# Pose-Group/FAMI-Pose

Hardware: AMD Instinct MI355X
Metric: train clips/sec (5-frame 384x288 HRNet-W48) (higher is better)
Workload: dtype f32

## Files before the change

fami-pose_amd/csrc/conv.hip:

```cpp
#include "common.h"
#include <type_traits>
#include <string.h>

#include "conv_epi.h"
#include "conv_pair.h"
extern "C" int fami_conv2d_fwd_bnin_ok(int N, int H, int W, int Ci, int Co);
extern "C" int fami_dcn_tune(int mode);
extern "C" int fami_bn_tune_small(long elems);
extern "C" void fami_conv_stem_tune(int on);
int fami_pair_launch(const PairCapture& c, hipStream_t s);
int fami_try_conv_stem1(int half_kind, const void* x, const void* wp, const float* bias, void* y, int N, int H, int W, int Ci, int Co,
                        int kh, int kw, int stride, int pad, int dil, int NTt, int relu, int accumulate, int out_f32, hipStream_t s,
                        const char* name, const EpiBN& epi);


struct ConvArgs {
  EpiBN e;
  int emode;
  const float* x;
  const float* wp;
  float* y;
  const float* bias;
  const float* addend;
  int N, Hi, Wi, Ci, Ho, Wo, Co;
// ... 589 lines not shown
  int xcd;
  int par;
};

template <typename H>
__global__ void pack_w_h_kernel(const float* __restrict__ w, H* __restrict__ wp, int Co, int Ci, int taps,
                                int KC, int NTt, int mode) {
  const long total = (long)taps * KC * NTt * 512;
  for (long i = blockIdx.x * (long)blockDim.x + threadIdx.x; i < total; i += (long)gridDim.x * blockDim.x) {
    const int j = (int)(i & 7), lane = (int)((i >> 3) & 63);
    long r = i >> 9;
    const int nt = (int)(r % NTt);
    r /= NTt;
    const int kc = (int)(r % KC), tap = (int)(r / KC);
    const int kidx = kc * 32 + (lane >> 4) * 8 + j, nidx = nt * 16 + (lane & 15);
    const int co = mode == 0 ? nidx : kidx, ci = mode == 0 ? kidx : nidx;
    float v = 0.f;
    if (co < Co && ci < Ci) v = w[((long)co * Ci + ci) * taps + tap];
    wp[i] = (H)v;
  }
}

struct PackDesc { long src, dst; int Co, Ci, taps, mode; };
template <typename T>
__global__ __launch_bounds__(256) void pack_w_batch_kernel(const float* __restrict__ params, T* __restrict__ packed,
                                                           const PackDesc* __restrict__ desc) {
  const PackDesc d = desc[blockIdx.y];
  const float* w = params + d.src;
  T* wp = packed + d.dst;
  const int kd = d.mode == 0 ? d.Ci : d.Co, nd = d.mode == 0 ? d.Co : d.Ci;
  constexpr int KG = sizeof(T) == 4 ? 16 : 32, FR = sizeof(T) == 4 ? 4 : 8;
  if (d.taps > 1 && d.taps <= 9) {
    __shared__ float tile[32 * (16 * 9 + 1) + 16];
    const int taps = d.taps;
    const int KC = (kd + KG - 1) / KG, NTt = (nd + 15) / 16;
    const int rows = d.mode == 0 ? 16 : KG, cols = d.mode == 0 ? KG : 16;
    const int run = cols * taps, pitch = run + 1;
    for (int b = blockIdx.x; b < KC * NTt; b += gridDim.x) {
      const int kc = b / NTt, nt = b - kc * NTt;
      const int co0 = d.mode == 0 ? nt * 16 : kc * KG, ci0 = d.mode == 0 ? kc * KG : nt * 16;
      __syncthreads();
      for (int i = threadIdx.x; i < rows * run; i += 256) {
        const int r = i / run, c = i - r * run;
        const int co = co0 + r, ci = ci0 + c / taps;
        tile[r * pitch + c] = (co < d.Co && ci < d.Ci) ? w[((long)co * d.Ci + ci0) * taps + c] : 0.f;
      }
      __syncthreads();
      for (int o = threadIdx.x; o < taps * 64 * FR; o += 256) {
        const int tap = o / (64 * FR), within = o - tap * (64 * FR);
        const int lane = within / FR, j = within - lane * FR;
        const int kl = (lane >> 4) * FR + j, nl = lane & 15;
        const int col = d.mode == 0 ? nl : kl, cil = d.mode == 0 ? kl : nl;
        st1(wp + ((long)(tap * KC + kc) * NTt + nt) * (64 * FR) + within, tile[col * pitch + cil * taps + tap]);
      }
    }
    return;
  }
  if constexpr (sizeof(T) == 4) {
    const long total = pack16_elems(kd, nd, d.taps) + pack32_elems(kd, nd, d.taps);
    for (long i = blockIdx.x * (long)blockDim.x + threadIdx.x; i < total; i += (long)gridDim.x * blockDim.x)
      st1(wp + i, pack_f32_elem(w, i, d.Co, d.Ci, d.taps, d.mode));
  } else {
    const int KC = (kd + KG - 1) / KG, NTt = (nd + 15) / 16;
    const long total = (long)d.taps * KC * NTt * 64 * FR;
    for (long i = blockIdx.x * (long)blockDim.x + threadIdx.x; i < total; i += (long)gridDim.x * blockDim.x) {
      const int j = (int)(i % FR), lane = (int)((i / FR) & 63);
      long r = i / (FR * 64);
      const int nt = (int)(r % NTt);
      r /= NTt;
      const int kc = (int)(r % KC), tap = (int)(r / KC);
      const int kidx = kc * KG + (lane >> 4) * FR + j, nidx = nt * 16 + (lane & 15);
      const int co = d.mode == 0 ? nidx : kidx, ci = d.mode == 0 ? kidx : nidx;
      float v = 0.f;
      if (co < d.Co && ci < d.Ci) v = w[((long)co * d.Ci + ci) * d.taps + tap];
      st1(wp + i, v);
    }
// ... 2314 lines not shown
  FAMI_REQUIRE(desc_out, nm, "null descriptor");
  EpiBN e = epi_none();
  if (slots) {
    FAMI_REQUIRE(epi_bwd_stats_ok(z, yrelu, mean, invstd, gamma, beta, relu), nm, "bad argument");
    e = epi_bwd_stats(slots, Ci, z, yrelu, mean, invstd, gamma, beta, relu);
  }
  return bwd_pair_run(
      nm, desc_out, s,
      [&] { return conv_dgrad_h_impl<HT>(nm, dy, wpd, dx, N, H, W, Ci, Co, kh, kw, stride, pad, dil, acc_dx, s, e); },
      [&] { return wgrad_h_impl<HT>(nm, x, dy, dw, workspace, ws_bytes, N, H, W, Ci, Co, kh, kw, stride, pad, dil, acc_dw, s); });
}

extern "C" {

int fami_conv_tune(int mt, int nt, int ks) {
  g_force_mt = mt; g_force_nt = nt; g_force_ks = ks;
  return FAMI_OK;
}
int fami_conv_tune_lds(int on) {
  if (on == 9000 || on == 9001) {
    fami_conv_stem_tune(on - 9000);
    return FAMI_OK;
  }
  if (on < 0) fami_conv_stem_tune(-1);
  if (on == 10 || on == 11 || on == 20 || on == 21 || on == 30 || on == 31 || (on >= 40 && on <= 42) || (on >= 52 && on <= 54) || (on >= 60 && on <= 62) || on >= 100) {
    fami_conv_t4_tune(on);
    return FAMI_OK;
  }
  g_use_lds = on < 0 ? -1 : (on ? 1 : 0);
  g_lds_sim = on == 2;
  if (on < 0) fami_conv_t4_tune(-1);
  return FAMI_OK;
}
int fami_conv_tune_wgrad_lds(int on) {
  if (on >= 30000) {
    fami_wgrad_s3_tune(on - 30000);
    return FAMI_OK;
  }
  if (on >= 20000) {
    fami_wgrad16_tune(on - 20000);
    return FAMI_OK;
  }
  if (on >= 1000) {
    g_wgrad_ps = on - 1000;
    return FAMI_OK;
  }
  if (on >= 50 && on <= 54) {
// ... 59 lines not shown
}

long fami_packed_weight_elems(int Co, int Ci, int kh, int kw, int mode) {
  const int kd = mode == 0 ? Ci : Co, nd = mode == 0 ? Co : Ci;
  return pack16_elems(kd, nd, kh * kw) + pack32_elems(kd, nd, kh * kw) + fami_split_image_elems(kd, nd, kh * kw);
}

int fami_pack_conv_weight_f32(const float* w_oihw, float* wp, int Co, int Ci, int kh, int kw, int mode,
                              hipStream_t s) {
  FAMI_REQUIRE(w_oihw && wp && Co > 0 && Ci > 0 && (mode == 0 || mode == 1), "fami_pack_conv_weight_f32", "bad argument");
  const int kd = mode == 0 ? Ci : Co, nd = mode == 0 ? Co : Ci;
  const long total = pack16_elems(kd, nd, kh * kw) + pack32_elems(kd, nd, kh * kw);
  hipLaunchKernelGGL(pack_w_kernel, dim3(fami_ew_grid(total)), dim3(256), 0, s, w_oihw, wp, Co, Ci, kh * kw, mode);
  FAMI_CHECK_LAUNCH("fami_pack_conv_weight_f32");
  if (fami_split_image_elems(kd, nd, kh * kw) > 0) {
    fami_pack_split_single(w_oihw, wp + total, Co, Ci, kh * kw, mode, s);
    FAMI_CHECK_LAUNCH("fami_pack_conv_weight_f32/split");
  }
  return FAMI_OK;
}

int fami_pack_conv_weights_batch_f32(const float* params, float* packed, const void* desc, int n, hipStream_t s) {
  FAMI_REQUIRE(params && packed && desc && n > 0 && n < 65536, "fami_pack_conv_weights_batch_f32", "bad argument");
  hipLaunchKernelGGL(pack_w_batch_kernel<float>, dim3(48, n), dim3(256), 0, s, params, packed, reinterpret_cast<const PackDesc*>(desc));
  FAMI_CHECK_LAUNCH("fami_pack_conv_weights_batch_f32");
  fami_pack_split_batch(params, packed, desc, n, s);
  FAMI_CHECK_LAUNCH("fami_pack_conv_weights_batch_f32/split");
  return FAMI_OK;
}

int fami_conv2d_fwd_f32(const float* x, const float* wp, const float* bias, const float* addend, float* y, int N,
                        int H, int W, int Ci, int Co, int kh, int kw, int stride, int pad, int dil, int relu,
                        int accumulate, hipStream_t s) {
  return conv_fwd_f32_impl("fami_conv2d_fwd_f32", x, wp, bias, addend, y, N, H, W, Ci, Co, kh, kw, stride, pad, dil, relu,
                           accumulate, epi_none(), s);
}
int fami_conv2d_fwd_stats_f32(const float* x, const float* wp, const float* bias, float* y, int N, int H, int W, int Ci,
                              int Co, int kh, int kw, int stride, int pad, int dil, void* slots, const float* pivot_src,
                              hipStream_t s) {
  FAMI_REQUIRE(slots, "fami_conv2d_fwd_stats_f32", "null slots");
  return conv_fwd_f32_impl("fami_conv2d_fwd_stats_f32", x, wp, bias, nullptr, y, N, H, W, Ci, Co, kh, kw, stride, pad, dil,
                           0, 0, epi_fwd_stats(slots, Co, pivot_src), s);
}
int fami_conv2d_fwd_xbn_f32(const float* z, const float* wp, const float* bias, float* y, int N, int H, int W, int Ci, int Co,
                            void* slots, const float* pivot_src, const void* xslots, long xP, const float* xgamma,
                            const float* xbeta, float* xmean, float* xinvstd, float* xrunning_mean, float* xrunning_var,
// ... 203 lines not shown
```

fami-pose_amd/csrc/conv_epi.h:

```cpp
#pragma once
#include "common.h"

struct EpiBN {
  double* slots;
  int ns, mode, relu, C;
  const float* pivot_src;
  const void* z;
  const void* yr;
  const float *mean, *invstd, *gamma, *beta;
};
static inline EpiBN epi_none() {
  EpiBN e;
  e.slots = nullptr; e.ns = 1; e.mode = 0; e.relu = 0; e.C = 0; e.pivot_src = nullptr; e.z = nullptr; e.yr = nullptr;
  e.mean = e.invstd = e.gamma = e.beta = nullptr;
  return e;
}
static inline EpiBN epi_fwd_stats(void* slots, int Co, const float* pivot_src) {
  EpiBN e = epi_none();
  if (!slots) return e;
  e.slots = reinterpret_cast<double*>(slots); e.ns = bn_slots(Co); e.mode = 1; e.C = Co; e.pivot_src = pivot_src;
  return e;
}
static inline bool epi_bwd_stats_ok(const void* z, const void* yrelu, const float* mean, const float* invstd, const float* gamma,
                                    const float* beta, int relu) {
// ... 97 lines not shown
int fami_try_conv3x3_t4(int half_kind, const void* x, const void* wp, const float* bias, void* y, int N, int H, int W, int Ci,
                        int Co, int KC, int NTt, int sgn, int relu, int accumulate, int out_f32, hipStream_t s,
                        const char* name, const EpiBN& epi, const XBN& xbn = xbn_none());
int fami_try_conv3x3_t4_dil(int half_kind, const void* x, const void* wp, const float* bias, void* y, int N, int H, int W, int Ci,
                            int Co, int KC, int NTt, int sgn, int relu, int accumulate, int out_f32, int dil, hipStream_t s,
                            const char* name);
void fami_conv_t4_tune(int on);
void fami_conv_t4_default_split(int on);
int fami_conv_t4_eligible16(int N, int H, int W, int Ci, int Co);
int fami_conv_t4_eligible_s3(int N, int H, int W, int Ci, int Co);

long fami_wgrad16_slabs(int N, int H, int W, int Ci, int Co, int k, int st, int pad, int dil);
int fami_try_wgrad16(int half_kind, const void* x, const void* dy, float* part, long ws_bytes, int N, int H, int W, int Ci,
                     int Co, int k, int st, int pad, int dil, hipStream_t s, const char* name, const XBN& xbn = xbn_none());
void fami_wgrad16_tune(int on);

long fami_wgrad_s3_slabs(int N, int H, int W, int Ci, int Co);
int fami_try_wgrad_s3(const float* x, const float* dy, float* part, long ws_bytes, int N, int H, int W, int Ci, int Co,
                      hipStream_t s, const char* name, const XBN& xbn = xbn_none());
void fami_wgrad_s3_tune(int on);
void fami_wgrad_s3_default(int on);

long fami_split_image_elems(int kd, int nd, int taps);
void fami_pack_split_single(const float* w_oihw, float* split, int Co, int Ci, int taps, int mode, hipStream_t s);
void fami_pack_split_batch(const float* params, float* packed, const void* desc, int n, hipStream_t s);
int fami_try_conv3x3_t5(int half_kind, const void* x, const void* wp, const float* bias, void* y, int N, int H, int W, int Ci,
                        int Co, int KC, int NTt, int sgn, int relu, int accumulate, int out_f32, hipStream_t s,
                        const char* name, const EpiBN& epi, const XBN& xbn);
void fami_conv_t5_tune(int on);
int fami_conv_t5_eligible_s3(int N, int H, int W, int Ci, int Co);

int fami_try_conv3x3_t6(int half_kind, const void* x, const void* wp, const float* bias, void* y, int N, int H, int W, int Ci,
                        int Co, int KC, int NTt, int sgn, int relu, int accumulate, int out_f32, hipStream_t s,
                        const char* name, const EpiBN& epi, const XBN& xbn);
extern "C" int fami_conv_t6_eligible(int N, int H, int W, int Ci, int Co);
void fami_conv_t6_tune(int on);
```

fami-pose_amd/csrc/conv_t5.hip:

```cpp
#include "conv_epi.h"
#include "conv_t5_dev.h"
#include "conv_pair.h"
#include <type_traits>


long fami_split_image_elems(int kd, int nd, int taps) {
  return (taps == 9 && kd % 16 == 0) ? (long)taps * (kd / 16) * ((nd + 15) / 16) * 384 : 0;
}
__device__ __forceinline__ void t5_split3(float v, __bf16& h0, __bf16& h1, __bf16& h2) {
  h0 = (__bf16)v;
  const float r1 = v - (float)h0;
  h1 = (__bf16)r1;
  const float r2 = r1 - (float)h1;
  h2 = (__bf16)r2;
}
struct T5PackDesc { long src, dst; int Co, Ci, taps, mode; };
__device__ __forceinline__ void t5_pack_split_image(const float* __restrict__ w, __bf16* __restrict__ sp, int Co, int Ci,
                                                    int mode, int first_block, int block_stride, float* tile) {
  const int kd = mode == 0 ? Ci : Co, nd = mode == 0 ? Co : Ci;
  const int KC = kd / 16, NTt = (nd + 15) / 16;
  constexpr int PITCH = 16 * 9 + 1;
  for (int b = first_block; b < KC * NTt; b += block_stride) {
    const int kc = b / NTt, nt = b - kc * NTt;
    const int co0 = mode == 0 ? nt * 16 : kc * 16, ci0 = mode == 0 ? kc * 16 : nt * 16;
    __syncthreads();
    for (int i = threadIdx.x; i < 16 * 144; i += 256) {
      const int r = i / 144, c = i - r * 144;
      const int co = co0 + r, ci = ci0 + c / 9;
      tile[r * PITCH + c] = (co < Co && ci < Ci) ? w[((long)co * Ci + ci0) * 9 + c] : 0.f;
    }
    __syncthreads();
    for (int o = threadIdx.x; o < 9 * 64; o += 256) {
      const int tap = o >> 6, n = (o >> 2) & 15, k4 = (o & 3) * 4;
      t5_bf16x4 h0, h1, h2;
#pragma unroll
      for (int j = 0; j < 4; ++j) {
        const int k = k4 + j;
        const float v = mode == 0 ? tile[n * PITCH + k * 9 + tap] : tile[k * PITCH + n * 9 + tap];
        __bf16 a0, a1, a2;
        t5_split3(v, a0, a1, a2);
        h0[j] = a0; h1[j] = a1; h2[j] = a2;
      }
      __bf16* blk = sp + ((long)(tap * KC + kc) * NTt + nt) * 768 + n * 16 + k4;
      *reinterpret_cast<t5_bf16x4*>(blk) = h0;
      *reinterpret_cast<t5_bf16x4*>(blk + 256) = h1;
      *reinterpret_cast<t5_bf16x4*>(blk + 512) = h2;
    }
  }
}
__global__ __launch_bounds__(256) void t5_pack_split_kernel(const float* __restrict__ w, __bf16* __restrict__ sp, int Co, int Ci, int mode) {
  __shared__ float tile[16 * (16 * 9 + 1)];
  t5_pack_split_image(w, sp, Co, Ci, mode, blockIdx.x, gridDim.x, tile);
}
__global__ __launch_bounds__(256) void t5_pack_split_batch_kernel(const float* __restrict__ params, float* __restrict__ packed,
                                                                   const T5PackDesc* __restrict__ desc) {
  __shared__ float tile[16 * (16 * 9 + 1)];
  const T5PackDesc d = desc[blockIdx.y];
  const int kd = d.mode == 0 ? d.Ci : d.Co, nd = d.mode == 0 ? d.Co : d.Ci;
  if (d.taps != 9 || (kd % 16) != 0) return;
  const long n16 = (long)9 * (kd / 16) * ((nd + 15) / 16) * 256;
  t5_pack_split_image(params + d.src, reinterpret_cast<__bf16*>(packed + d.dst + n16), d.Co, d.Ci, d.mode, blockIdx.x, gridDim.x, tile);
}
void fami_pack_split_single(const float* w_oihw, float* split, int Co, int Ci, int taps, int mode, hipStream_t s) {
  const int kd = mode == 0 ? Ci : Co, nd = mode == 0 ? Co : Ci;
  if (fami_split_image_elems(kd, nd, taps) == 0) return;
  int blocks = (kd / 16) * ((nd + 15) / 16);
  if (blocks > 512) blocks = 512;
  hipLaunchKernelGGL(t5_pack_split_kernel, dim3(blocks), dim3(256), 0, s, w_oihw, reinterpret_cast<__bf16*>(split), Co, Ci, mode);
}
void fami_pack_split_batch(const float* params, float* packed, const void* desc, int n, hipStream_t s) {
// ... 148 lines not shown
```

fami-pose_amd/csrc/conv_t5_dev.h:

```cpp
#pragma once
#include "conv_epi.h"
#include <type_traits>
typedef __bf16 t5_bf16x4 __attribute__((ext_vector_type(4)));

struct ConvT5Args {
  EpiBN e;
  int emode;
  XBN xb;
  const void* x;
  const void* wimg;
  void* y;
  const float* bias;
  int N, H, W, Ci, Co;
  int R, bands, cblocks, njobs;
  int PW, KC, NTt;
  int sgn, relu, accumulate, out_f32;
  int ppl;
  int patch_bytes;
  int nposmax;
  int abl_chunks;
  long long* dbg;
};

#define T5_THREADS 512
#define T5_WAVES 8
#define T5_MTT 3
// ... 481 lines not shown
```

fami-pose_amd/csrc/norm.hip:

```cpp
#include "common.h"

#define BN_MAXG 512
#ifndef BN_U
#define BN_U 4
#endif

struct ColMap {
  int cv, prow, rows, CV;
  bool active;
};
__device__ __forceinline__ ColMap col_map(int C) {
  ColMap m;
  m.CV = C >> 2;
  m.rows = 256 / m.CV;
  m.cv = threadIdx.x % m.CV;
  m.prow = threadIdx.x / m.CV;
  m.active = m.prow < m.rows;
  return m;
}

__device__ __forceinline__ double block_sum_d(double v, double* sm4) {
  v = wave_sum_d(v);
  const int lane = threadIdx.x & 63, wave = threadIdx.x >> 6;
  __syncthreads();
// ... 188 lines not shown
__device__ __forceinline__ f32x4 bn_relu_mask(f32x4 g, f32x4 yy) {
#pragma unroll
  for (int t = 0; t < 4; ++t) g[t] = yy[t] > 0.f ? g[t] : 0.f;
  return g;
}
__device__ __forceinline__ f32x4 bn_relu_mask(f32x4 g, int relu, f32x4 yy, f32x4 xv, f32x4 sc, f32x4 sf) {
  if (relu == 1) return bn_relu_mask(g, yy);
  if (relu == 2) {
#pragma unroll
    for (int t = 0; t < 4; ++t) g[t] = __builtin_fmaf(xv[t], sc[t], sf[t]) > 0.f ? g[t] : 0.f;
  }
  return g;
}

__device__ __forceinline__ void bn_load_stats(const float* __restrict__ mean, const float* __restrict__ invstd, int c0, f32x4& mu,
                                              f32x4& is) {
#pragma unroll
  for (int t = 0; t < 4; ++t) {
    mu[t] = mean[c0 + t];
    is[t] = invstd[c0 + t];
  }
}

template <typename T>
__device__ __forceinline__ void bn_bwd_sums(const T* __restrict__ dy, const T* __restrict__ x, const T* __restrict__ y,
                                            const ColMap& m, long P, int C, int relu, f32x4 mu, f32x4 is, f32x4 sc, f32x4 sf,
                                            f32x4& s, f32x4& q) {
  const long step = (long)gridDim.x * m.rows;
  for (long p = (long)blockIdx.x * m.rows + m.prow; p < P; p += BN_U * step) {
    f32x4 g[BN_U], yy[BN_U], xx[BN_U];
    long o[BN_U];
#pragma unroll
    for (int u = 0; u < BN_U; ++u) {
      const long pu = p + u * step;
      o[u] = (pu < P ? pu : p) * C + m.cv * 4;
      g[u] = ld4(dy + o[u]);
    }
    if (relu & 1) {
#pragma unroll
      for (int u = 0; u < BN_U; ++u) yy[u] = ld4(y + o[u]);
    }
#pragma unroll
    for (int u = 0; u < BN_U; ++u) xx[u] = ld4(x + o[u]);
#pragma unroll
    for (int u = 0; u < BN_U; ++u) {
      if (relu == 1) g[u] = bn_relu_mask(g[u], yy[u]);
      if (relu == 2) g[u] = bn_relu_mask(g[u], relu, yy[u], xx[u], sc, sf);
      if (p + u * step >= P) g[u] = f32x4{0.f, 0.f, 0.f, 0.f};
      const f32x4 xh = (xx[u] - mu) * is;
      s += g[u];
      q += g[u] * xh;
    }
  }
}

template <typename T>
__global__ __launch_bounds__(256) void bn_bwd_partial_kernel(const T* __restrict__ dy,
                                                             const T* __restrict__ x,
                                                             const T* __restrict__ y,
                                                             const float* __restrict__ mean,
                                                             const float* __restrict__ invstd,
                                                             float* __restrict__ partial, long P, int C, int relu) {
  extern __shared__ float sm[];
  const ColMap m = col_map(C);
  f32x4 s = {0.f, 0.f, 0.f, 0.f}, q = {0.f, 0.f, 0.f, 0.f};
  if (m.active) {
    f32x4 mu, is;
    bn_load_stats(mean, invstd, m.cv * 4, mu, is);
    const f32x4 none = {0.f, 0.f, 0.f, 0.f};
    bn_bwd_sums(dy, x, y, m, P, C, relu ? 1 : 0, mu, is, none, none, s, q);
    bn_stage_rows(sm, m, C, s, q);
  }
  bn_fold_rows<false>(sm, m.rows, C, partial, nullptr, 0);
}

__global__ void bn_bwd_finalize_kernel(const float* __restrict__ partial, int G, long P, int C, float* coef,
                                       float* dgamma, float* dbeta, int accumulate) {
  __shared__ double sm4[4];
  const int c = blockIdx.x;
  double s = 0.0, q = 0.0;
  for (int g = threadIdx.x; g < G; g += 256) {
    s += (double)partial[(long)g * 2 * C + c];
    q += (double)partial[(long)g * 2 * C + C + c];
  }
  s = block_sum_d(s, sm4);
  q = block_sum_d(q, sm4);
  if (threadIdx.x != 0) return;
  if (coef) {
    coef[c] = (float)(s / (double)P);
    coef[C + c] = (float)(q / (double)P);
  }
  if (dgamma) dgamma[c] = accumulate ? dgamma[c] + (float)q : (float)q;
  if (dbeta) dbeta[c] = accumulate ? dbeta[c] + (float)s : (float)s;
// ... 148 lines not shown
    bn_scale_shift(muf, isf, gamma[c], beta[c], sc, sf);
    sm[c] = sc;
    sm[C + c] = sf;
  }
  __syncthreads();
  const ColMap m = col_map(C);
  if (!m.active) return;
  const f32x4 sc = *reinterpret_cast<const f32x4*>(sm + m.cv * 4), sf = *reinterpret_cast<const f32x4*>(sm + C + m.cv * 4);
  for (long p = (long)blockIdx.x * m.rows + m.prow; p < P; p += (long)gridDim.x * m.rows) {
    const long o = p * C + m.cv * 4;
    const f32x4 xv = ld4(x + o);
    f32x4 v;
#pragma unroll
    for (int t = 0; t < 4; ++t) v[t] = __builtin_fmaf(xv[t], sc[t], sf[t]);
    if (residual) v += ld4(residual + o);
    if (relu) {
#pragma unroll
      for (int t = 0; t < 4; ++t) v[t] = fmaxf(v[t], 0.f);
    }
    st4(y + o, v);
  }
}

template <typename T>
__global__ __launch_bounds__(256) void bn_bwd_partial2_kernel(const T* __restrict__ dy, const T* __restrict__ x,
                                                              const T* __restrict__ y, const float* __restrict__ mean,
                                                              const float* __restrict__ invstd,
                                                              const float* __restrict__ gamma,
                                                              const float* __restrict__ beta,
                                                              double* __restrict__ slots, int NS, long P, int C, int relu) {
  extern __shared__ float sm[];
  const ColMap m = col_map(C);
  f32x4 s = {0.f, 0.f, 0.f, 0.f}, q = {0.f, 0.f, 0.f, 0.f};
  if (m.active) {
    f32x4 mu, is, sc, sf;
    bn_load_stats(mean, invstd, m.cv * 4, mu, is);
#pragma unroll
    for (int t = 0; t < 4; ++t) {
      float a, b;
      bn_scale_shift(mu[t], is[t], gamma[m.cv * 4 + t], beta[m.cv * 4 + t], a, b);
      sc[t] = a;
      sf[t] = b;
    }
    bn_bwd_sums(dy, x, y, m, P, C, relu, mu, is, sc, sf, s, q);
    bn_stage_rows(sm, m, C, s, q);
  }
  bn_fold_rows<true>(sm, m.rows, C, nullptr, slots, NS);
}

template <typename T>
__global__ __launch_bounds__(256) void bn_bwd_apply2_kernel(const T* __restrict__ dy, const T* __restrict__ x,
                                                            const T* __restrict__ y, const float* __restrict__ mean,
                                                            const float* __restrict__ invstd,
                                                            const float* __restrict__ gamma,
                                                            const float* __restrict__ beta,
                                                            const double* __restrict__ slots, int NS, T* __restrict__ dx,
                                                            float* dgamma, float* dbeta, T* __restrict__ dres, long P,
                                                            int C, int relu, int acc_dx, int acc_param, int acc_dres) {
  extern __shared__ float sm[];
  for (int c = threadIdx.x; c < C; c += 256) {
    double s, q;
    bn_fold_slots(slots, NS, C, c, s, q);
    sm[c] = (float)(s / (double)P);
    sm[C + c] = (float)(q / (double)P);
    if (blockIdx.x == 0) {
      if (dgamma) dgamma[c] = acc_param ? dgamma[c] + (float)q : (float)q;
      if (dbeta) dbeta[c] = acc_param ? dbeta[c] + (float)s : (float)s;
// ... 194 lines not shown
  out[c] = accumulate ? out[c] + (float)s : (float)s;
}

static inline int bn_rows(int C) { return 256 / (C >> 2); }
static inline int bn_capped_grid(long P, int C, int steps, long cap) {
  const long per = (long)bn_rows(C) * steps;
  long g = (P + per - 1) / per;
  if (g > cap) g = cap;
  if (g < 1) g = 1;
  return (int)g;
}
static inline int bn_grid(long P, int C) { return bn_capped_grid(P, C, 2 * BN_U, BN_MAXG); }
static inline int bn_grid2(long P, int C, int esz) {
  return bn_capped_grid(P, C, 2 * BN_U, (long)g_bn2_maxg * (esz == 4 ? 4 : 1));
}
static inline int bn_apply_grid(long P, int C) { return bn_capped_grid(P, C, 1, 2048); }
static inline int bn_apply_grid2(long P, int C) { return bn_capped_grid(P, C, 1, 1024); }
static inline int bn_check_shape(long P, int C, const char* nm) {
  if (P > 0 && C >= 4 && (C % 4) == 0 && C <= 1024) return FAMI_OK;
  fami_set_error(nm, "C must be a multiple of 4, <= 1024");
  return FAMI_ESHAPE;
}

static inline size_t bn_stage_bytes(int C) { return (size_t)bn_rows(C) * 2 * C * sizeof(float); }

template <typename T>
static int bn_small_fwd_launch(const T* x, const T* residual, T* y, const float* gamma, const float* beta, float* mean,
                               float* invstd, float* running_mean, float* running_var, long P, int C, int relu,
                               float momentum, float eps, hipStream_t s, const char* nm) {
  hipLaunchKernelGGL(bn_small_fwd_kernel<T>, dim3(C / 4), dim3(256), 0, s, x, residual, y, gamma, beta, mean, invstd,
                     running_mean, running_var, P, C, relu, momentum, eps);
  FAMI_CHECK_LAUNCH(nm);
  return FAMI_OK;
}
template <typename T>
static int bn_small_bwd_launch(const T* dy, const T* x, const T* y, const float* mean, const float* invstd,
                               const float* gamma, T* dx, float* dgamma, float* dbeta, T* dres, long P, int C, int relu,
                               int acc_dx, int acc_param, int acc_dres, hipStream_t s, const char* nm) {
  hipLaunchKernelGGL(bn_small_bwd_kernel<T>, dim3(C / 4), dim3(256), 0, s, dy, x, y, mean, invstd, gamma, dx, dgamma,
                     dbeta, dres, P, C, relu, acc_dx, acc_param, acc_dres);
  FAMI_CHECK_LAUNCH(nm);
  return FAMI_OK;
}

template <typename T>
static int bn_stats_impl(const T* x, long P, int C, float* mean, float* invstd, float* running_mean,
// ... 12 lines not shown
template <typename T>
static int bn_apply_impl(const T* x, const float* mean, const float* invstd, const float* gamma, const float* beta,
                         const T* residual, T* y, long P, int C, int relu, hipStream_t s, const char* nm) {
  FAMI_REQUIRE(x && mean && invstd && gamma && beta && y, nm, "null pointer");
  if (const int rc = bn_check_shape(P, C, nm)) return rc;
  hipLaunchKernelGGL(bn_apply_kernel<T>, dim3(bn_apply_grid(P, C)), dim3(256), 0, s, x, mean, invstd, gamma, beta, residual, y, P,
                     C, relu);
  FAMI_CHECK_LAUNCH(nm);
  return FAMI_OK;
}

template <typename T>
static int bn_bwd_impl(const T* dy, const T* x, const T* y, const float* mean, const float* invstd,
                       const float* gamma, T* dx, float* dgamma, float* dbeta, T* dres, long P, int C, int relu,
                       int acc_dx, int acc_param, int acc_dres, float* ws, hipStream_t s, const char* nm) {
  FAMI_REQUIRE(dy && x && mean && invstd && gamma && dx && ws, nm, "null pointer");
  FAMI_REQUIRE(!relu || y, nm, "relu needs y");
  if (const int rc = bn_check_shape(P, C, nm)) return rc;
  if (bn_small_ok(P, C))
    return bn_small_bwd_launch<T>(dy, x, y, mean, invstd, gamma, dx, dgamma, dbeta, dres, P, C, relu, acc_dx, acc_param, acc_dres, s, nm);
  const int G = bn_grid(P, C);
  float* coef = ws + (long)BN_MAXG * 2 * C - 2 * C;
  const int Gp = G < BN_MAXG ? G : BN_MAXG - 1;
  hipLaunchKernelGGL(bn_bwd_partial_kernel<T>, dim3(Gp), dim3(256), bn_stage_bytes(C), s, dy, x, y, mean, invstd, ws, P,
                     C, relu);
  FAMI_CHECK_LAUNCH(nm);
  hipLaunchKernelGGL(bn_bwd_finalize_kernel, dim3(C), dim3(256), 0, s, ws, Gp, P, C, coef, dgamma, dbeta, acc_param);
  FAMI_CHECK_LAUNCH(nm);
  hipLaunchKernelGGL(bn_bwd_apply_kernel<T>, dim3(bn_apply_grid(P, C)), dim3(256), 0, s, dy, x, y, mean, invstd, gamma, coef, dx,
                     dres, P, C, relu, acc_dx, acc_dres);
  FAMI_CHECK_LAUNCH(nm);
  return FAMI_OK;
}

template <typename T>
static int bn_eval_bwd_impl(const T* dy, const T* x, const T* y, const float* mean, const float* invstd,
                            const float* gamma, T* dx, float* dgamma, float* dbeta, T* dres, long P, int C, int relu,
                            int acc_dx, int acc_param, int acc_dres, float* ws, hipStream_t s, const char* nm) {
  FAMI_REQUIRE(dy && invstd && gamma && dx, nm, "null pointer");
  FAMI_REQUIRE(!relu || y, nm, "relu needs y");
  if (const int rc = bn_check_shape(P, C, nm)) return rc;
  if (!dgamma && !dbeta) {
    hipLaunchKernelGGL((bn_eval_bwd_kernel<T, false>), dim3(bn_capped_grid(P, C, BN_U, 2048)), dim3(256), 0, s, dy, x, y, mean, invstd, gamma,
                       (float*)nullptr, dx, dres, P, C, relu, acc_dx, acc_dres);
    FAMI_CHECK_LAUNCH(nm);
    return FAMI_OK;
  }
  FAMI_REQUIRE(x && mean && ws, nm, "parameter sums need x, mean and ws");
// ... 34 lines not shown
                       P, C);
    FAMI_CHECK_LAUNCH(nm);
  }
  hipLaunchKernelGGL(bn_apply2_kernel<T>, dim3(bn_apply_grid2(P, C)), dim3(256), (size_t)2 * C * sizeof(float), s, x,
                     reinterpret_cast<const double*>(slots), NS, gamma, beta, residual, y, mean, invstd, running_mean,
                     running_var, P, C, relu, momentum, eps, pre ? bn_slots_pivot(slots, C) : (const float*)nullptr);
  FAMI_CHECK_LAUNCH(nm);
  return FAMI_OK;
}

template <typename T>
static int bn_bwd2_impl(const T* dy, const T* x, const T* y, const float* mean, const float* invstd, const float* gamma,
                        const float* beta, T* dx, float* dgamma, float* dbeta, T* dres, long P, int C, int relu,
                        int acc_dx, int acc_param, int acc_dres, void* slots, int pre, hipStream_t s, const char* nm) {
  FAMI_REQUIRE(dy && x && mean && invstd && gamma && beta && dx && slots, nm, "null pointer");
  FAMI_REQUIRE(relu != 1 || y, nm, "relu = 1 needs y");
  FAMI_REQUIRE(relu >= 0 && relu <= 2, nm, "relu must be 0, 1 (mask from y) or 2 (mask recomputed from x)");
  if (const int rc = bn_check_shape(P, C, nm)) return rc;
  if (bn_small_ok(P, C) && !pre) {
    FAMI_REQUIRE(relu != 2 || y, nm, "small tensors take the ReLU mask from y");
    return bn_small_bwd_launch<T>(dy, x, y, mean, invstd, gamma, dx, dgamma, dbeta, dres, P, C, relu ? 1 : 0, acc_dx, acc_param, acc_dres, s, nm);
  }
  const int G = bn_grid2(P, C, (int)sizeof(T)), NS = bn_slots(C);
  if (!pre) {
    hipLaunchKernelGGL(bn_bwd_partial2_kernel<T>, dim3(G), dim3(256), bn_stage_bytes(C), s, dy, x, y, mean, invstd, gamma, beta,
                       reinterpret_cast<double*>(slots), NS, P, C, relu);
    FAMI_CHECK_LAUNCH(nm);
  }
  hipLaunchKernelGGL(bn_bwd_apply2_kernel<T>, dim3(bn_apply_grid2(P, C)), dim3(256), (size_t)2 * C * sizeof(float), s, dy, x,
                     y, mean, invstd, gamma, beta, reinterpret_cast<const double*>(slots), NS, dx, dgamma, dbeta, dres, P,
                     C, relu, acc_dx, acc_param, acc_dres);
  FAMI_CHECK_LAUNCH(nm);
  return FAMI_OK;
}

template <typename T>
static int channel_sum_impl(const T* x, long P, int C, float* out, int accumulate, float* ws, hipStream_t s,
                            const char* nm) {
  FAMI_REQUIRE(x && out && ws && P > 0 && C > 0, nm, "bad argument");
  FAMI_REQUIRE(C <= 4096, nm, "C > 4096 unsupported");
  int rows = C > 256 ? 1 : 256 / C;
  const bool vec4 = C % 4 == 0 && C <= 1024 && P >= 4096;
  if (vec4) rows = bn_rows(C);
  long g = (P + rows - 1) / rows;
  if (vec4) g = (g + 2 * BN_U - 1) / (2 * BN_U);
  if (g > BN_MAXG) g = BN_MAXG;
  if (g < 1) g = 1;
  if (vec4) hipLaunchKernelGGL(chan_sum_partial4_kernel<T>, dim3((int)g), dim3(256), (size_t)rows * C * sizeof(float), s, x, ws, P, C);
  else hipLaunchKernelGGL(chan_sum_partial_kernel<T>, dim3((int)g), dim3(256), C > 256 ? 0 : (size_t)rows * C * sizeof(float), s, x, ws, P, C);
  FAMI_CHECK_LAUNCH(nm);
  hipLaunchKernelGGL(chan_sum_finalize_kernel, dim3(C), dim3(256), 0, s, ws, (int)g, C, out, accumulate);
  FAMI_CHECK_LAUNCH(nm);
  return FAMI_OK;
}

extern "C" {

long fami_bn_workspace(int C) { return (long)BN_MAXG * 2 * C * (long)sizeof(float); }
long fami_bn_slots_bytes(int C) { return bn_slots_bytes(C); }
int fami_bn_tune_small(long elems) {
  if (elems <= -1000) { g_bn2_maxg = (int)(-elems - 1000); return FAMI_OK; }
  if (elems < 0) { g_bn_small_elems = 32768; g_bn2_maxg = 512; return FAMI_OK; }
  g_bn_small_elems = elems;
  return FAMI_OK;
}
int fami_bn_is_small(long P, int C) { return bn_small_ok(P, C) ? 1 : 0; }
long fami_channel_sum_workspace(int C) { return (long)BN_MAXG * C * (long)sizeof(float); }

int fami_bn_eval_stats_f32(const float* running_mean, const float* running_var, float* mean, float* invstd, int C,
                           float eps, hipStream_t s) {
  FAMI_REQUIRE(running_mean && running_var && mean && invstd && C > 0, "fami_bn_eval_stats_f32", "bad argument");
  hipLaunchKernelGGL(bn_eval_stats_kernel, dim3(fami_cdiv(C, 64)), dim3(64), 0, s, running_mean, running_var, mean,
                     invstd, C, eps);
  FAMI_CHECK_LAUNCH("fami_bn_eval_stats_f32");
  return FAMI_OK;
}

int fami_bn_finalize_slots_f32(void* slots, long P, int C, float* mean, float* invstd, float* running_mean,
                               float* running_var, float momentum, float eps, hipStream_t s) {
  FAMI_REQUIRE(slots && mean && invstd && C > 0 && P > 0, "fami_bn_finalize_slots_f32", "bad argument");
  hipLaunchKernelGGL(bn_finalize_slots_kernel, dim3(fami_cdiv(C, 64)), dim3(64), 0, s, reinterpret_cast<const double*>(slots),
                     bn_slots(C), bn_slots_pivot(slots, C), P, C, mean, invstd, running_mean, running_var, momentum, eps);
  FAMI_CHECK_LAUNCH("fami_bn_finalize_slots_f32");
  return FAMI_OK;
}
// ... 109 lines not shown
```

fami-pose_amd/csrc/route.h:

```cpp
#pragma once
#include "../../include/fami_route.h"
extern "C" fami_route_t* fami_rt(void);

#define g_dcn_gather (fami_rt()->dcn_gather)
#define g_dcn_abl (fami_rt()->dcn_abl)
#define g_dcn_win_r (fami_rt()->dcn_win_r)
#define g_dcn_ksplit (fami_rt()->dcn_ksplit)
#define g_dcn_pf (fami_rt()->dcn_pf)
#define g_dcn_bwd2 (fami_rt()->dcn_bwd2)
#define g_dcn_bwd2_cap (fami_rt()->dcn_bwd2_cap)
#define g_dcn_bwd2_stage (fami_rt()->dcn_bwd2_stage)
#define g_dcn_bwd_abl (fami_rt()->dcn_bwd_abl)
#define g_dcn_bwd_scatter (fami_rt()->dcn_bwd_scatter)
#define g_prio (fami_rt()->prio)
#define g_lin_conv (fami_rt()->lin_conv)
#define g_par (fami_rt()->par)
#define g_force_mt (fami_rt()->force_mt)
#define g_force_nt (fami_rt()->force_nt)
#define g_force_ks (fami_rt()->force_ks)
#define g_stages (fami_rt()->stages)
#define g_use32 (fami_rt()->use32)
#define g_xcd_w (fami_rt()->xcd_w)
#define g_xcd (fami_rt()->xcd)
#define g_use_lds (fami_rt()->use_lds)
// ... 39 lines not shown
#define g_wg6_s2 (fami_rt()->wg6_s2)
#define g_wg6_dil (fami_rt()->wg6_dil)
#define g_wg6_c42 (fami_rt()->wg6_c42)
#define g_wg6_c4 (fami_rt()->wg6_c4)
#define g_wg6 (fami_rt()->wg6)
#define g_wg6_nu (fami_rt()->wg6_nu)
#define g_wg6_target (fami_rt()->wg6_target)
#define g_wg6_target_c4 (fami_rt()->wg6_target_c4)
#define g_wg1 (fami_rt()->wg1)
#define g_wg1_target (fami_rt()->wg1_target)
#define g_wgs (fami_rt()->wgs)
#define g_wg16_abl (fami_rt()->wg16_abl)
#define g_wg16 (fami_rt()->wg16)
#define g_wg16_bt (fami_rt()->wg16_bt)
#define g_wg16_target (fami_rt()->wg16_target)
#define g_wg16_general (fami_rt()->wg16_general)
#define g_wg16_bt18 (fami_rt()->wg16_bt18)
#define g_wgs3 (fami_rt()->wgs3)
#define g_wgs3_bt (fami_rt()->wgs3_bt)
#define g_wgs3_target (fami_rt()->wgs3_target)
#define g_wgs3_default (fami_rt()->wgs3_default)
#define g_bn_small_elems (fami_rt()->bn_small_elems)
#define g_bn2_maxg (fami_rt()->bn2_maxg)

static inline void fami_route_set_dcn_defaults(fami_route_t* q) {
  q->dcn_gather = -1;
  q->dcn_abl = 0;
  q->dcn_win_r = 0;
  q->dcn_ksplit = 1;
  q->dcn_pf = 0;
  q->dcn_bwd2 = 1;
  q->dcn_bwd2_cap = 36;
  q->dcn_bwd2_stage = 1;
  q->dcn_bwd_abl = 0;
  q->dcn_bwd_scatter = -1;
}

static inline void fami_route_set_defaults(fami_route_t* q) {
  q->size = (int)sizeof(fami_route_t);
  fami_route_set_dcn_defaults(q);
  q->prio = 0;
  q->lin_conv = 1;
  q->par = 1;
  q->force_mt = 0;
  q->force_nt = 0;
  q->force_ks = 0;
// ... 44 lines not shown
  q->wg6_s2 = 1;
  q->wg6_dil = 1;
  q->wg6_c42 = 1;
  q->wg6_c4 = 1;
  q->wg6 = 1;
  q->wg6_nu = 0;
  q->wg6_target = 80;
  q->wg6_target_c4 = 160;
  q->wg1 = 1;
  q->wg1_target = 192;
  q->wgs = 1;
  q->wg16_abl = 0;
  q->wg16 = 1;
  q->wg16_bt = 0;
  q->wg16_target = 0;
  q->wg16_general = 1;
  q->wg16_bt18 = 0;
  q->wgs3 = 1;
  q->wgs3_bt = 0;
  q->wgs3_target = 0;
  q->wgs3_default = 1;
  q->bn_small_elems = 32768;
  q->bn2_maxg = 512;
}
```

include/fami_route.h:

```cpp
#ifndef FAMI_ROUTE_H
#define FAMI_ROUTE_H
#ifdef __cplusplus
extern "C" {
#endif

typedef struct fami_route_t {
  int size;
  int  dcn_gather;
  int  dcn_abl;
  int  dcn_win_r;
  int  dcn_ksplit;
  int  dcn_pf;
  int  dcn_bwd2;
  int  dcn_bwd2_cap;
  int  dcn_bwd2_stage;
  int  dcn_bwd_abl;
  int  dcn_bwd_scatter;
  int  prio;
  int  lin_conv;
  int  par;
  int  force_mt;
  int  force_nt;
  int  force_ks;
  int  stages;
// ... 43 lines not shown
  int  wg6_s2;
  int  wg6_dil;
  int  wg6_c42;
  int  wg6_c4;
  int  wg6;
  int  wg6_nu;
  int  wg6_target;
  int  wg6_target_c4;
  int  wg1;
  int  wg1_target;
  int  wgs;
  int  wg16_abl;
  int  wg16;
  int  wg16_bt;
  int  wg16_target;
  int  wg16_general;
  int  wg16_bt18;
  int  wgs3;
  int  wgs3_bt;
  int  wgs3_target;
  int  wgs3_default;
  long bn_small_elems;
  int  bn2_maxg;
} fami_route_t;

#ifdef __cplusplus
}
#endif
#endif
```

Measured before the change: 92.00.

## Fuse bf16 split packing into weight pack and write BN relu-masked grad early

Two unrelated fusions, both on by default. First, the batched f32 weight-pack kernel now also writes the three-way bf16 split image for 3x3 weights from its shared-memory tile, so the separate split-pack launch and its reread of the weights go away. Second, the BN backward partial-sum kernel, when a residual-gradient buffer is present and does not overlap the other buffers, stores the relu-masked gradient into that buffer. The apply pass then reads it in place of dy and y. This cuts one input stream and the relu recomputation in the apply pass at the cost of an extra write in the partial pass.

Result: no change. 92.77 (median of 6 runs) (+0.8%).

```diff
diff --git a/fami-pose_amd/csrc/conv.hip b/fami-pose_amd/csrc/conv.hip
--- a/fami-pose_amd/csrc/conv.hip
+++ b/fami-pose_amd/csrc/conv.hip
@@ -635,7 +635,7 @@
 }
 
 struct PackDesc { long src, dst; int Co, Ci, taps, mode; };
-template <typename T>
+template <typename T, bool SPLIT = false>
 __global__ __launch_bounds__(256) void pack_w_batch_kernel(const float* __restrict__ params, T* __restrict__ packed,
                                                            const PackDesc* __restrict__ desc) {
   const PackDesc d = desc[blockIdx.y];
@@ -665,6 +665,11 @@
         const int kl = (lane >> 4) * FR + j, nl = lane & 15;
         const int col = d.mode == 0 ? nl : kl, cil = d.mode == 0 ? kl : nl;
         st1(wp + ((long)(tap * KC + kc) * NTt + nt) * (64 * FR) + within, tile[col * pitch + cil * taps + tap]);
+      }
+      if constexpr (SPLIT && sizeof(T) == 4) {
+        if (taps == 9 && (kd % 16) == 0)
+          t5_split_block(tile, pitch, d.mode, reinterpret_cast<__bf16*>(wp + (long)9 * KC * NTt * 256) + ((long)kc * NTt + nt) * 768,
+                         (long)KC * NTt * 768);
       }
     }
     return;
@@ -3025,7 +3030,11 @@
     fami_conv_stem_tune(on - 9000);
     return FAMI_OK;
   }
-  if (on < 0) fami_conv_stem_tune(-1);
+  if (on == 9010 || on == 9011) {
+    g_pack_fused = on - 9010;
+    return FAMI_OK;
+  }
+  if (on < 0) { fami_conv_stem_tune(-1); g_pack_fused = 1; }
   if (on == 10 || on == 11 || on == 20 || on == 21 || on == 30 || on == 31 || (on >= 40 && on <= 42) || (on >= 52 && on <= 54) || (on >= 60 && on <= 62) || on >= 100) {
     fami_conv_t4_tune(on);
     return FAMI_OK;
@@ -3131,6 +3140,11 @@
 
 int fami_pack_conv_weights_batch_f32(const float* params, float* packed, const void* desc, int n, hipStream_t s) {
   FAMI_REQUIRE(params && packed && desc && n > 0 && n < 65536, "fami_pack_conv_weights_batch_f32", "bad argument");
+  if (g_pack_fused) {
+    hipLaunchKernelGGL((pack_w_batch_kernel<float, true>), dim3(48, n), dim3(256), 0, s, params, packed, reinterpret_cast<const PackDesc*>(desc));
+    FAMI_CHECK_LAUNCH("fami_pack_conv_weights_batch_f32");
+    return FAMI_OK;
+  }
   hipLaunchKernelGGL(pack_w_batch_kernel<float>, dim3(48, n), dim3(256), 0, s, params, packed, reinterpret_cast<const PackDesc*>(desc));
   FAMI_CHECK_LAUNCH("fami_pack_conv_weights_batch_f32");
   fami_pack_split_batch(params, packed, desc, n, s);
diff --git a/fami-pose_amd/csrc/conv_epi.h b/fami-pose_amd/csrc/conv_epi.h
--- a/fami-pose_amd/csrc/conv_epi.h
+++ b/fami-pose_amd/csrc/conv_epi.h
@@ -143,6 +143,32 @@
 void fami_wgrad_s3_default(int on);
 
 long fami_split_image_elems(int kd, int nd, int taps);
+typedef __bf16 t5_bf16x4 __attribute__((ext_vector_type(4)));
+__device__ __forceinline__ void t5_split3(float v, __bf16& h0, __bf16& h1, __bf16& h2) {
+  h0 = (__bf16)v;
+  const float r1 = v - (float)h0;
+  h1 = (__bf16)r1;
+  const float r2 = r1 - (float)h1;
+  h2 = (__bf16)r2;
+}
+__device__ __forceinline__ void t5_split_block(const float* tile, int pitch, int mode, __bf16* __restrict__ blk0, long tap_stride) {
+  for (int o = threadIdx.x; o < 9 * 64; o += 256) {
+    const int tap = o >> 6, n = (o >> 2) & 15, k4 = (o & 3) * 4;
+    t5_bf16x4 h0, h1, h2;
+#pragma unroll
+    for (int j = 0; j < 4; ++j) {
+      const int k = k4 + j;
+      const float v = mode == 0 ? tile[n * pitch + k * 9 + tap] : tile[k * pitch + n * 9 + tap];
+      __bf16 a0, a1, a2;
+      t5_split3(v, a0, a1, a2);
+      h0[j] = a0; h1[j] = a1; h2[j] = a2;
+    }
+    __bf16* blk = blk0 + tap * tap_stride + n * 16 + k4;
+    *reinterpret_cast<t5_bf16x4*>(blk) = h0;
+    *reinterpret_cast<t5_bf16x4*>(blk + 256) = h1;
+    *reinterpret_cast<t5_bf16x4*>(blk + 512) = h2;
+  }
+}
 void fami_pack_split_single(const float* w_oihw, float* split, int Co, int Ci, int taps, int mode, hipStream_t s);
 void fami_pack_split_batch(const float* params, float* packed, const void* desc, int n, hipStream_t s);
 int fami_try_conv3x3_t5(int half_kind, const void* x, const void* wp, const float* bias, void* y, int N, int H, int W, int Ci,
diff --git a/fami-pose_amd/csrc/conv_t5.hip b/fami-pose_amd/csrc/conv_t5.hip
--- a/fami-pose_amd/csrc/conv_t5.hip
+++ b/fami-pose_amd/csrc/conv_t5.hip
@@ -6,13 +6,6 @@
 
 long fami_split_image_elems(int kd, int nd, int taps) {
   return (taps == 9 && kd % 16 == 0) ? (long)taps * (kd / 16) * ((nd + 15) / 16) * 384 : 0;
-}
-__device__ __forceinline__ void t5_split3(float v, __bf16& h0, __bf16& h1, __bf16& h2) {
-  h0 = (__bf16)v;
-  const float r1 = v - (float)h0;
-  h1 = (__bf16)r1;
-  const float r2 = r1 - (float)h1;
-  h2 = (__bf16)r2;
 }
 struct T5PackDesc { long src, dst; int Co, Ci, taps, mode; };
 __device__ __forceinline__ void t5_pack_split_image(const float* __restrict__ w, __bf16* __restrict__ sp, int Co, int Ci,
@@ -30,22 +23,7 @@
       tile[r * PITCH + c] = (co < Co && ci < Ci) ? w[((long)co * Ci + ci0) * 9 + c] : 0.f;
     }
     __syncthreads();
-    for (int o = threadIdx.x; o < 9 * 64; o += 256) {
-      const int tap = o >> 6, n = (o >> 2) & 15, k4 = (o & 3) * 4;
-      t5_bf16x4 h0, h1, h2;
-#pragma unroll
-      for (int j = 0; j < 4; ++j) {
-        const int k = k4 + j;
-        const float v = mode == 0 ? tile[n * PITCH + k * 9 + tap] : tile[k * PITCH + n * 9 + tap];
-        __bf16 a0, a1, a2;
-        t5_split3(v, a0, a1, a2);
-        h0[j] = a0; h1[j] = a1; h2[j] = a2;
-      }
-      __bf16* blk = sp + ((long)(tap * KC + kc) * NTt + nt) * 768 + n * 16 + k4;
-      *reinterpret_cast<t5_bf16x4*>(blk) = h0;
-      *reinterpret_cast<t5_bf16x4*>(blk + 256) = h1;
-      *reinterpret_cast<t5_bf16x4*>(blk + 512) = h2;
-    }
+    t5_split_block(tile, PITCH, mode, sp + ((long)kc * NTt + nt) * 768, (long)KC * NTt * 768);
   }
 }
 __global__ __launch_bounds__(256) void t5_pack_split_kernel(const float* __restrict__ w, __bf16* __restrict__ sp, int Co, int Ci, int mode) {
diff --git a/fami-pose_amd/csrc/conv_t5_dev.h b/fami-pose_amd/csrc/conv_t5_dev.h
--- a/fami-pose_amd/csrc/conv_t5_dev.h
+++ b/fami-pose_amd/csrc/conv_t5_dev.h
@@ -1,7 +1,6 @@
 #pragma once
 #include "conv_epi.h"
 #include <type_traits>
-typedef __bf16 t5_bf16x4 __attribute__((ext_vector_type(4)));
 
 struct ConvT5Args {
   EpiBN e;
diff --git a/fami-pose_amd/csrc/norm.hip b/fami-pose_amd/csrc/norm.hip
--- a/fami-pose_amd/csrc/norm.hip
+++ b/fami-pose_amd/csrc/norm.hip
@@ -234,10 +234,10 @@
   }
 }
 
-template <typename T>
+template <typename T, bool DZ = false>
 __device__ __forceinline__ void bn_bwd_sums(const T* __restrict__ dy, const T* __restrict__ x, const T* __restrict__ y,
                                             const ColMap& m, long P, int C, int relu, f32x4 mu, f32x4 is, f32x4 sc, f32x4 sf,
-                                            f32x4& s, f32x4& q) {
+                                            f32x4& s, f32x4& q, T* __restrict__ dz_out = nullptr) {
   const long step = (long)gridDim.x * m.rows;
   for (long p = (long)blockIdx.x * m.rows + m.prow; p < P; p += BN_U * step) {
     f32x4 g[BN_U], yy[BN_U], xx[BN_U];
@@ -259,6 +259,7 @@
       if (relu == 1) g[u] = bn_relu_mask(g[u], yy[u]);
       if (relu == 2) g[u] = bn_relu_mask(g[u], relu, yy[u], xx[u], sc, sf);
       if (p + u * step >= P) g[u] = f32x4{0.f, 0.f, 0.f, 0.f};
+      else if (DZ) st4(dz_out + o[u], g[u]);
       const f32x4 xh = (xx[u] - mu) * is;
       s += g[u];
       q += g[u] * xh;
@@ -266,13 +267,14 @@
   }
 }
 
-template <typename T>
+template <typename T, bool DZ>
 __global__ __launch_bounds__(256) void bn_bwd_partial_kernel(const T* __restrict__ dy,
                                                              const T* __restrict__ x,
                                                              const T* __restrict__ y,
                                                              const float* __restrict__ mean,
                                                              const float* __restrict__ invstd,
-                                                             float* __restrict__ partial, long P, int C, int relu) {
+                                                             float* __restrict__ partial, long P, int C, int relu,
+                                                             T* __restrict__ dz_out) {
   extern __shared__ float sm[];
   const ColMap m = col_map(C);
   f32x4 s = {0.f, 0.f, 0.f, 0.f}, q = {0.f, 0.f, 0.f, 0.f};
@@ -280,7 +282,7 @@
     f32x4 mu, is;
     bn_load_stats(mean, invstd, m.cv * 4, mu, is);
     const f32x4 none = {0.f, 0.f, 0.f, 0.f};
-    bn_bwd_sums(dy, x, y, m, P, C, relu ? 1 : 0, mu, is, none, none, s, q);
+    bn_bwd_sums<T, DZ>(dy, x, y, m, P, C, relu ? 1 : 0, mu, is, none, none, s, q, dz_out);
     bn_stage_rows(sm, m, C, s, q);
   }
   bn_fold_rows<false>(sm, m.rows, C, partial, nullptr, 0);
@@ -475,13 +477,14 @@
   }
 }
 
-template <typename T>
+template <typename T, bool DZ>
 __global__ __launch_bounds__(256) void bn_bwd_partial2_kernel(const T* __restrict__ dy, const T* __restrict__ x,
                                                               const T* __restrict__ y, const float* __restrict__ mean,
                                                               const float* __restrict__ invstd,
                                                               const float* __restrict__ gamma,
                                                               const float* __restrict__ beta,
-                                                              double* __restrict__ slots, int NS, long P, int C, int relu) {
+                                                              double* __restrict__ slots, int NS, long P, int C, int relu,
+                                                              T* __restrict__ dz_out) {
   extern __shared__ float sm[];
   const ColMap m = col_map(C);
   f32x4 s = {0.f, 0.f, 0.f, 0.f}, q = {0.f, 0.f, 0.f, 0.f};
@@ -495,7 +498,7 @@
       sc[t] = a;
       sf[t] = b;
     }
-    bn_bwd_sums(dy, x, y, m, P, C, relu, mu, is, sc, sf, s, q);
+    bn_bwd_sums<T, DZ>(dy, x, y, m, P, C, relu, mu, is, sc, sf, s, q, dz_out);
     bn_stage_rows(sm, m, C, s, q);
   }
   bn_fold_rows<true>(sm, m.rows, C, nullptr, slots, NS);
@@ -736,6 +739,15 @@
   return FAMI_ESHAPE;
 }
 
+template <typename T>
+static inline bool bn_dz_form(const T* dy, const T* x, const T* y, const T* dx, const T* dres, long P, int C, int relu, int acc_dres) {
+  if (!g_bn_bwd_dz || relu != 1 || !dres || acc_dres) return false;
+  const uintptr_t n = (uintptr_t)P * C * sizeof(T), r = (uintptr_t)dres;
+  for (const T* t : {dy, x, y, dx})
+    if (t && (uintptr_t)t < r + n && r < (uintptr_t)t + n) return false;
+  return true;
+}
+
 static inline size_t bn_stage_bytes(int C) { return (size_t)bn_rows(C) * 2 * C * sizeof(float); }
 
 template <typename T>
@@ -794,8 +806,14 @@
   const int G = bn_grid(P, C);
   float* coef = ws + (long)BN_MAXG * 2 * C - 2 * C;
   const int Gp = G < BN_MAXG ? G : BN_MAXG - 1;
-  hipLaunchKernelGGL(bn_bwd_partial_kernel<T>, dim3(Gp), dim3(256), bn_stage_bytes(C), s, dy, x, y, mean, invstd, ws, P,
-                     C, relu);
+  if (bn_dz_form(dy, x, y, dx, dres, P, C, relu ? 1 : 0, acc_dres)) {
+    hipLaunchKernelGGL((bn_bwd_partial_kernel<T, true>), dim3(Gp), dim3(256), bn_stage_bytes(C), s, dy, x, y, mean, invstd, ws, P,
+                       C, relu, dres);
+    dy = dres, y = nullptr, dres = nullptr, relu = 0;
+  } else {
+    hipLaunchKernelGGL((bn_bwd_partial_kernel<T, false>), dim3(Gp), dim3(256), bn_stage_bytes(C), s, dy, x, y, mean, invstd, ws, P,
+                       C, relu, (T*)nullptr);
+  }
   FAMI_CHECK_LAUNCH(nm);
   hipLaunchKernelGGL(bn_bwd_finalize_kernel, dim3(C), dim3(256), 0, s, ws, Gp, P, C, coef, dgamma, dbeta, acc_param);
   FAMI_CHECK_LAUNCH(nm);
@@ -876,9 +894,14 @@
     return bn_small_bwd_launch<T>(dy, x, y, mean, invstd, gamma, dx, dgamma, dbeta, dres, P, C, relu ? 1 : 0, acc_dx, acc_param, acc_dres, s, nm);
   }
   const int G = bn_grid2(P, C, (int)sizeof(T)), NS = bn_slots(C);
-  if (!pre) {
-    hipLaunchKernelGGL(bn_bwd_partial2_kernel<T>, dim3(G), dim3(256), bn_stage_bytes(C), s, dy, x, y, mean, invstd, gamma, beta,
-                       reinterpret_cast<double*>(slots), NS, P, C, relu);
+  if (!pre && bn_dz_form(dy, x, y, dx, dres, P, C, relu, acc_dres)) {
+    hipLaunchKernelGGL((bn_bwd_partial2_kernel<T, true>), dim3(G), dim3(256), bn_stage_bytes(C), s, dy, x, y, mean, invstd, gamma, beta,
+                       reinterpret_cast<double*>(slots), NS, P, C, relu, dres);
+    FAMI_CHECK_LAUNCH(nm);
+    dy = dres, y = nullptr, dres = nullptr, relu = 0;
+  } else if (!pre) {
+    hipLaunchKernelGGL((bn_bwd_partial2_kernel<T, false>), dim3(G), dim3(256), bn_stage_bytes(C), s, dy, x, y, mean, invstd, gamma, beta,
+                       reinterpret_cast<double*>(slots), NS, P, C, relu, (T*)nullptr);
     FAMI_CHECK_LAUNCH(nm);
   }
   hipLaunchKernelGGL(bn_bwd_apply2_kernel<T>, dim3(bn_apply_grid2(P, C)), dim3(256), (size_t)2 * C * sizeof(float), s, dy, x,
@@ -914,7 +937,8 @@
 long fami_bn_slots_bytes(int C) { return bn_slots_bytes(C); }
 int fami_bn_tune_small(long elems) {
   if (elems <= -1000) { g_bn2_maxg = (int)(-elems - 1000); return FAMI_OK; }
-  if (elems < 0) { g_bn_small_elems = 32768; g_bn2_maxg = 512; return FAMI_OK; }
+  if (elems == -900 || elems == -901) { g_bn_bwd_dz = (int)(-elems - 900); return FAMI_OK; }
+  if (elems < 0) { g_bn_small_elems = 32768; g_bn2_maxg = 512; g_bn_bwd_dz = 1; return FAMI_OK; }
   g_bn_small_elems = elems;
   return FAMI_OK;
 }
diff --git a/fami-pose_amd/csrc/route.h b/fami-pose_amd/csrc/route.h
--- a/fami-pose_amd/csrc/route.h
+++ b/fami-pose_amd/csrc/route.h
@@ -85,6 +85,8 @@
 #define g_wgs3_default (fami_rt()->wgs3_default)
 #define g_bn_small_elems (fami_rt()->bn_small_elems)
 #define g_bn2_maxg (fami_rt()->bn2_maxg)
+#define g_bn_bwd_dz (fami_rt()->bn_bwd_dz)
+#define g_pack_fused (fami_rt()->pack_fused)
 
 static inline void fami_route_set_dcn_defaults(fami_route_t* q) {
   q->dcn_gather = -1;
@@ -175,4 +177,6 @@
   q->wgs3_default = 1;
   q->bn_small_elems = 32768;
   q->bn2_maxg = 512;
+  q->bn_bwd_dz = 1;
+  q->pack_fused = 1;
 }
diff --git a/include/fami_route.h b/include/fami_route.h
--- a/include/fami_route.h
+++ b/include/fami_route.h
@@ -89,6 +89,8 @@
   int  wgs3_default;
   long bn_small_elems;
   int  bn2_maxg;
+  int  bn_bwd_dz;
+  int  pack_fused;
 } fami_route_t;
 
 #ifdef __cplusplus
```
